# gaetanfacchinetti/DensityFlows.jl

Measured on AMD Instinct MI355X. Metric: forward+logdetJ Msamples/s, d=5 8-layer RealNVP, 1/2/4/8 MI355X, higher is better.
Workload: dtype f32

## Files before the change

### densityflows.jl_amd/csrc/df_uniform_impl.h

```cpp
#pragma once

#include <type_traits>

#include "df_chain_impl.h"

namespace df {
namespace uni {


using impl::lds4;
using impl::mfma4;
using impl::Stager;

__device__ __forceinline__ float relu_fast(float x) {
    return __int_as_float(__builtin_elementwise_max(__float_as_int(x), 0));
}

__device__ __forceinline__ float xgroup_sum(float p) {
    auto a = __builtin_amdgcn_permlane16_swap(__float_as_uint(p), __float_as_uint(p), false, false);
    const float q = __uint_as_float(a[0]) + __uint_as_float(a[1]);
    auto b = __builtin_amdgcn_permlane32_swap(__float_as_uint(q), __float_as_uint(q), false, false);
    return __uint_as_float(b[0]) + __uint_as_float(b[1]);
}


template <int HT, int TT, int KS = 0>
__device__ __forceinline__ void dense_first(const uint8_t* buf, const UNet& N, const float (&xin)[TT][4],
                                            f32x4 (&acc)[TT][HT]) {
    const int lane = threadIdx.x & 63;
    const float* wb = reinterpret_cast<const float*>(buf + N.off_w0) + lane;
    const int ks = KS > 0 ? KS : N.ks;
    if constexpr (KS > 0) {
#pragma unroll
        for (int m = 0; m < HT; ++m) {
            const float w = wb[m * KS * 64];
#pragma unroll
            for (int t = 0; t < TT; ++t) acc[t][m] = mfma4(w, xin[t][0], f32x4{0.f, 0.f, 0.f, 0.f});
        }
#pragma unroll
        for (int r = 1; r < KS; ++r)
#pragma unroll
            for (int m = 0; m < HT; ++m) {
                const float w = wb[(m * KS + r) * 64];
#pragma unroll
                for (int t = 0; t < TT; ++t) acc[t][m] = mfma4(w, xin[t][r], acc[t][m]);
            }
        return;
    }
#pragma unroll
    for (int t = 0; t < TT; ++t)
#pragma unroll
        for (int m = 0; m < HT; ++m) acc[t][m] = f32x4{0.f, 0.f, 0.f, 0.f};
#pragma unroll
    for (int r = 0; r < 4; ++r) {
        if (r < ks) {
#pragma unroll
            for (int m = 0; m < HT; ++m) {
                const float w = wb[(m * ks + r) * 64];
#pragma unroll
                for (int t = 0; t < TT; ++t) acc[t][m] = mfma4(w, xin[t][r], acc[t][m]);
            }
        }
    }
}

template <int HT, int TT>
__device__ __forceinline__ void dense_hidden(const uint8_t* wb, const f32x4 (&in)[TT][HT], f32x4 (&out)[TT][HT]) {
    const int lane = threadIdx.x & 63;
    wb += lane * 16;
    constexpr int MB = HT < 2 ? HT : 2;
#pragma unroll
    for (int t = 0; t < TT; ++t)
#pragma unroll
        for (int m = 0; m < HT; ++m) out[t][m] = f32x4{0.f, 0.f, 0.f, 0.f};
#pragma unroll
    for (int m0 = 0; m0 < HT; m0 += MB) {
        f32x4 w[2][MB];
#pragma unroll
        for (int mm = 0; mm < MB; ++mm) w[0][mm] = lds4(wb + (m0 + mm) * 1024);
#pragma unroll
        for (int kq = 0; kq < HT; ++kq) {
            const int cb = kq & 1;
            if (kq + 1 < HT) {
#pragma unroll
                for (int mm = 0; mm < MB; ++mm) w[cb ^ 1][mm] = lds4(wb + ((kq + 1) * HT + m0 + mm) * 1024);
            }
#pragma unroll
            for (int r = 0; r < 4; ++r)
#pragma unroll
                for (int mm = 0; mm < MB; ++mm)
#pragma unroll
                    for (int t = 0; t < TT; ++t)
                        out[t][m0 + mm] = mfma4(w[cb][mm][r], in[t][kq][r], out[t][m0 + mm]);
        }
    }
}

template <int HT, int TT, bool RELU>
__device__ __forceinline__ void bias_act(const uint8_t* bb, int act, f32x4 (&v)[TT][HT], bool add_bias = true) {
    const int g = (threadIdx.x & 63) >> 4;
    if (add_bias) {
#pragma unroll
        for (int m = 0; m < HT; ++m) {
            const f32x4 b = lds4(bb + ((16 * m + 4 * g) << 2));
#pragma unroll
            for (int t = 0; t < TT; ++t) v[t][m] = v[t][m] + b;
        }
    }
    if (RELU || act == DF_ACT_RELU) {
#pragma unroll
        for (int t = 0; t < TT; ++t)
#pragma unroll
            for (int m = 0; m < HT; ++m)
#pragma unroll
                for (int r = 0; r < 4; ++r) v[t][m][r] = relu_fast(v[t][m][r]);
    } else if (act != DF_ACT_IDENTITY) {
        if (!RELU) {
#pragma unroll
            for (int t = 0; t < TT; ++t)
#pragma unroll
                for (int m = 0; m < HT; ++m)
#pragma unroll
                    for (int r = 0; r < 4; ++r) v[t][m][r] = impl::act_fn(act, v[t][m][r]);
        }
    }
}

template <int HT, int TT, bool RELU, int NO = 0>
__device__ __forceinline__ void out_valu(const uint8_t* buf, const UNet& N, const f32x4 (&h)[TT][HT],
                                         f32x4 (&o)[TT]) {
    const int g = (threadIdx.x & 63) >> 4;
    const uint8_t* w3 = buf + N.off_out;
    constexpr int INP = 16 * HT;
    const int n_out = NO > 0 ? NO : N.n_out;
    const float* b3 = reinterpret_cast<const float*>(w3) + n_out * INP;
#pragma unroll
    for (int t = 0; t < TT; ++t) o[t] = f32x4{0.f, 0.f, 0.f, 0.f};
#pragma unroll
    for (int oo = 0; oo < 4; ++oo) {
        if (oo < n_out) {
            float p[TT];
#pragma unroll
            for (int t = 0; t < TT; ++t) p[t] = 0.f;
#pragma unroll
            for (int kq = 0; kq < HT; ++kq) {
                const f32x4 w = lds4(w3 + ((oo * INP + 16 * kq + 4 * g) << 2));
#pragma unroll
                for (int r = 0; r < 4; ++r)
#pragma unroll
                    for (int t = 0; t < TT; ++t) p[t] = __builtin_fmaf(w[r], h[t][kq][r], p[t]);
            }
            const float bo = b3[oo];
#pragma unroll
            for (int t = 0; t < TT; ++t) {
                const float v = xgroup_sum(p[t]) + bo;
                o[t][oo] = (RELU || N.act_out == DF_ACT_IDENTITY) ? v : impl::act_fn(N.act_out, v);
            }
        }
    }
}

template <int HT, int TT, int NO>
__device__ __forceinline__ void out_valu_t(const uint8_t* buf, const UNet& N, const f32x4 (&h)[TT][HT],
                                           float (&y)[TT]) {
    static_assert(NO >= 1 && NO <= 4, "FAST tails: 1..4 outputs");
    const int g = (threadIdx.x & 63) >> 4;
    const uint8_t* w3 = buf + N.off_out;
    constexpr int INP = 16 * HT;
    float p[TT][4];
#pragma unroll
    for (int t = 0; t < TT; ++t)
#pragma unroll
        for (int oo = 0; oo < 4; ++oo) p[t][oo] = 0.f;
#pragma unroll
    for (int oo = 0; oo < NO; ++oo)
#pragma unroll
        for (int kq = 0; kq < HT; ++kq) {
            const f32x4 w = lds4(w3 + ((oo * INP + 16 * kq + 4 * g) << 2));
#pragma unroll
            for (int r = 0; r < 4; ++r)
#pragma unroll
                for (int t = 0; t < TT; ++t) p[t][oo] = __builtin_fmaf(w[r], h[t][kq][r], p[t][oo]);
        }
    const float bo = reinterpret_cast<const float*>(w3)[NO * INP + (g < NO ? g : 0)];
#pragma unroll
    for (int t = 0; t < TT; ++t) {
        auto a = __builtin_amdgcn_permlane16_swap(__float_as_uint(p[t][0]), __float_as_uint(p[t][1]), false, false);
        const float A = __uint_as_float(a[0]) + __uint_as_float(a[1]);
        float Bv = 0.f;
        if constexpr (NO > 2) {
            auto b = __builtin_amdgcn_permlane16_swap(__float_as_uint(p[t][2]), __float_as_uint(p[t][3]), false, false);
            Bv = __uint_as_float(b[0]) + __uint_as_float(b[1]);
        }
        auto c = __builtin_amdgcn_permlane32_swap(__float_as_uint(A), __float_as_uint(Bv), false, false);
        y[t] = (__uint_as_float(c[0]) + __uint_as_float(c[1])) + bo;
    }
}

template <int NO>
__device__ __forceinline__ float group_row_sum(float y) {
    float s = y;
    if constexpr (NO > 1) {
        auto a = __builtin_amdgcn_permlane16_swap(__float_as_uint(y), __float_as_uint(y), false, false);
        s = s + __uint_as_float(a[1]);
    }
    if constexpr (NO > 2) {
        auto b = __builtin_amdgcn_permlane32_swap(__float_as_uint(y), __float_as_uint(y), false, false);
        const float y2 = __uint_as_float(b[1]);
        s = s + y2;
        if constexpr (NO > 3) {
            auto c = __builtin_amdgcn_permlane16_swap(__float_as_uint(y2), __float_as_uint(y2), false, false);
            s = s + __uint_as_float(c[1]);
        }
    }
    return s;
}

template <int HT, int TT, bool RELU>
__device__ __forceinline__ void out_mfma(const uint8_t* buf, const UNet& N, const f32x4 (&h)[TT][HT],
                                         f32x4 (&out)[TT][2]) {
    const int lane = threadIdx.x & 63, g = lane >> 4;
    const uint8_t* wb = buf + N.off_out + lane * 16;
    const int mt = (N.n_out + 15) >> 4;
#pragma unroll
    for (int t = 0; t < TT; ++t) out[t][0] = out[t][1] = f32x4{0.f, 0.f, 0.f, 0.f};
#pragma unroll
    for (int kq = 0; kq < HT; ++kq) {
        const f32x4 w0 = lds4(wb + (kq * mt + 0) * 1024);
#pragma unroll
        for (int r = 0; r < 4; ++r)
#pragma unroll
            for (int t = 0; t < TT; ++t) out[t][0] = mfma4(w0[r], h[t][kq][r], out[t][0]);
        if (mt > 1) {
            const f32x4 w1 = lds4(wb + (kq * mt + 1) * 1024);
#pragma unroll
            for (int r = 0; r < 4; ++r)
#pragma unroll
                for (int t = 0; t < TT; ++t) out[t][1] = mfma4(w1[r], h[t][kq][r], out[t][1]);
        }
    }
    const uint8_t* bb = buf + N.off_out + HT * mt * 1024;
#pragma unroll
    for (int m = 0; m < 2; ++m) {
        if (m < mt) {
            const f32x4 b = lds4(bb + ((16 * m + 4 * g) << 2));
#pragma unroll
            for (int t = 0; t < TT; ++t) {
                f32x4 v = out[t][m] + b;
                if (!RELU && N.act_out != DF_ACT_IDENTITY)
#pragma unroll
                    for (int r = 0; r < 4; ++r) v[r] = impl::act_fn(N.act_out, v[r]);
                out[t][m] = v;
            }
        }
    }
}

template <int PH>
__device__ __forceinline__ float couple1(float v, float y) {
    if (PH == impl::PH_S_FWD) return v * expf(y);
    if (PH == impl::PH_T_FWD) return v + y;
    if (PH == impl::PH_T_BWD) return v - y;
    return v * expf(-y);
}

template <int HT, int TT, bool OUTV, bool RELU, int PH, int NO = 0>
__device__ __forceinline__ void tail(const uint8_t* buf, const UNet& N, const ULayer& L, const int32_t* tab,
                                     float* state, const int (&ro)[TT], float (&sum)[TT], const f32x4 (&H)[TT][HT]) {
    const int g = (threadIdx.x & 63) >> 4;
    constexpr bool SPH = (PH == impl::PH_S_FWD || PH == impl::PH_S_BWD);
    const int32_t* af = tab + L.af_tab;
    const int n_af = (OUTV && NO > 0) ? NO : L.n_af;
#pragma unroll
    for (int t = 0; t < TT; ++t) sum[t] = 0.f;
#ifdef DF_EXP_NOTAIL
    if (true) {
#pragma unroll
        for (int t = 0; t < TT; ++t) {
            float acc = 0.f;
#pragma unroll
            for (int m = 0; m < HT; ++m) acc += H[t][m][0];
            asm volatile("" ::"v"(acc));
        }
        return;
    }
#endif
    if constexpr (OUTV && NO > 0) {
        float y[TT];
        out_valu_t<HT, TT, NO>(buf, N, H, y);
        const int slot = af[g < NO ? g : 0];
#pragma unroll
        for (int t = 0; t < TT; ++t) {
            if (g < NO) state[ro[t] + slot] = couple1<PH>(state[ro[t] + slot], y[t]);
            if (SPH) sum[t] = group_row_sum<NO>(y[t]);
        }
    } else if constexpr (OUTV) {
        f32x4 o[TT];
        out_valu<HT, TT, RELU, NO>(buf, N, H, o);
        const int slot = (g < n_af) ? af[g] : 0;
#pragma unroll
        for (int t = 0; t < TT; ++t) {
            const float y = impl::sel4(o[t], g);
            if (g < n_af) state[ro[t] + slot] = couple1<PH>(state[ro[t] + slot], y);
            if (SPH) {
                float s_ = o[t][0];
#pragma unroll
                for (int oo = 1; oo < 4; ++oo)
                    if (oo < n_af) s_ = s_ + o[t][oo];
                sum[t] = s_;
            }
        }
    } else {
        f32x4 o[TT][2];
        out_mfma<HT, TT, RELU>(buf, N, H, o);
#pragma unroll
        for (int t = 0; t < TT; ++t) {
            float p = 0.f;
#pragma unroll
            for (int m = 0; m < 2; ++m)
#pragma unroll
                for (int r = 0; r < 4; ++r) {
                    const int oo = 16 * m + 4 * g + r;
                    if (oo < L.n_af) {
                        const int slot = af[oo];
                        const float y = o[t][m][r];
                        state[ro[t] + slot] = couple1<PH>(state[ro[t] + slot], y);
                        if (SPH) p = p + y;
                    }
                }
            if (SPH) sum[t] = xgroup_sum(p);
        }
    }
}

typedef __bf16 bf16x8 __attribute__((ext_vector_type(8)));

__device__ __forceinline__ f32x4 mfma_bf(const bf16x8& a, const bf16x8& b, f32x4 c) {
    return __builtin_amdgcn_mfma_f32_16x16x32_bf16(a, b, c, 0, 0, 0);
}

typedef __bf16 bf16x2 __attribute__((ext_vector_type(2)));
#ifndef DF_SPLIT_DOT2
#define DF_SPLIT_DOT2 1
#endif
template <int S>
__device__ __forceinline__ float split_rem(bf16x2 h, float x) {
#if DF_SPLIT_DOT2 == 2
    const uint32_t u = __builtin_bit_cast(uint32_t, h);
    const float hi = __uint_as_float(S == 0 ? (u << 16) : (u & 0xffff0000u));
    float r;
    asm("v_sub_f32 %0, %1, %2" : "=v"(r) : "v"(x), "v"(hi));
    return r;
#elif DF_SPLIT_DOT2
    uint32_t c;
    if (S == 0) asm("v_mov_b32 %0, 0xbf80" : "=v"(c));
    else c = 0xbf800000u;
    return __builtin_amdgcn_fdot2_f32_bf16(h, __builtin_bit_cast(bf16x2, c), x, false);
#else
    return x - (float)h[S];
#endif
}

__device__ __forceinline__ void split2(float a, float b, bf16x2& p0, bf16x2& p1, bf16x2& p2) {
    p0 = bf16x2{(__bf16)a, (__bf16)b};
    const float ra = split_rem<0>(p0, a), rb = split_rem<1>(p0, b);
    p1 = bf16x2{(__bf16)ra, (__bf16)rb};
    p2 = bf16x2{(__bf16)split_rem<0>(p1, ra), (__bf16)split_rem<1>(p1, rb)};
}

__device__ __forceinline__ void split8(const float (&v)[8], bf16x8& p0, bf16x8& p1, bf16x8& p2) {
#pragma unroll
    for (int e = 0; e < 8; e += 2) {
        bf16x2 h, m, l;
        split2(v[e], v[e + 1], h, m, l);
        p0[e] = h[0]; p0[e + 1] = h[1];
        p1[e] = m[0]; p1[e + 1] = m[1];
        p2[e] = l[0]; p2[e + 1] = l[1];
    }
}

#ifndef DF_SPLIT_MREM
#define DF_SPLIT_MREM 1
#endif
typedef short short4v __attribute__((ext_vector_type(4)));
typedef __bf16 bf16x4v __attribute__((ext_vector_type(4)));

__device__ __forceinline__ short4v neg_eye() {
    const int i = threadIdx.x & 3;
    short4v p;
#pragma unroll
    for (int e = 0; e < 4; ++e) p[e] = (e == i) ? (short)0xbf80 : (short)0;
    return p;
}

__device__ __forceinline__ f32x4 mrem(short4v eye, bf16x4v h, f32x4 c) {
    return __builtin_amdgcn_mfma_f32_4x4x4bf16_1k(eye, __builtin_bit_cast(short4v, h), c, 0, 0, 0);
}

__device__ __forceinline__ void split8_mrem(short4v eye, const f32x4& a, const f32x4& b, bf16x8& p0, bf16x8& p1,
                                            bf16x8& p2) {
    bf16x4v h0, h1;
#pragma unroll
    for (int e = 0; e < 4; ++e) {
        h0[e] = (__bf16)a[e];
        h1[e] = (__bf16)b[e];
    }
    p0 = __builtin_shufflevector(h0, h1, 0, 1, 2, 3, 4, 5, 6, 7);
    const f32x4 ra = mrem(eye, h0, a), rb = mrem(eye, h1, b);
#pragma unroll
    for (int e = 0; e < 4; ++e) {
        h0[e] = (__bf16)ra[e];
        h1[e] = (__bf16)rb[e];
    }
    p1 = __builtin_shufflevector(h0, h1, 0, 1, 2, 3, 4, 5, 6, 7);
    const f32x4 sa = mrem(eye, h0, ra), sb = mrem(eye, h1, rb);
#pragma unroll
    for (int e = 0; e < 4; ++e) {
        h0[e] = (__bf16)sa[e];
        h1[e] = (__bf16)sb[e];
    }
    p2 = __builtin_shufflevector(h0, h1, 0, 1, 2, 3, 4, 5, 6, 7);
}

template <int HT, int TT>
__device__ __forceinline__ void dense_first_split(const uint8_t* buf, const UNet& N, const float (&xin)[TT][4],
                                                  f32x4 (&acc)[TT][HT]) {
    const int lane = threadIdx.x & 63;
    bf16x8 b[TT];
    const __bf16 z = (__bf16)0.f;
#pragma unroll
    for (int t = 0; t < TT; t += 2) {
        bf16x2 h, m, l;
        split2(xin[t][0], t + 1 < TT ? xin[t + 1][0] : 0.f, h, m, l);
        b[t] = bf16x8{h[0], m[0], h[0], l[0], m[0], h[0], z, z};
        if (t + 1 < TT) b[t + 1] = bf16x8{h[1], m[1], h[1], l[1], m[1], h[1], z, z};
    }
    const uint8_t* wb = buf + N.off_w0 + lane * 16;
#pragma unroll
    for (int m = 0; m < HT; ++m) {
        const bf16x8 w = *reinterpret_cast<const bf16x8*>(wb + m * 1024);
#pragma unroll
        for (int t = 0; t < TT; ++t) acc[t][m] = mfma_bf(w, b[t], f32x4{0.f, 0.f, 0.f, 0.f});
    }
}

template <int HT, int TT, bool BIAS = true, bool FENCE = false>
__device__ __forceinline__ void dense_hidden_split(const uint8_t* wb, const f32x4 (&in)[TT][HT],
                                                   f32x4 (&out)[TT][HT]) {
    const int lane = threadIdx.x & 63, g = lane >> 4;
    const uint8_t* bb = wb + (HT / 2) * HT * 3072;
    wb += lane * 16;
    const short4v eye = DF_SPLIT_MREM ? neg_eye() : short4v{0, 0, 0, 0};
#pragma unroll
    for (int m = 0; m < HT; ++m) {
        const f32x4 b = BIAS ? lds4(bb + ((16 * m + 4 * g) << 2)) : f32x4{0.f, 0.f, 0.f, 0.f};
#pragma unroll
        for (int t = 0; t < TT; ++t) out[t][m] = b;
    }
#pragma unroll
    for (int c = 0; c < HT / 2; ++c) {
        bf16x8 x[TT][3];
#pragma unroll
        for (int t = 0; t < TT; ++t) {
            const float v[8] = {in[t][2 * c][0],     in[t][2 * c][1],     in[t][2 * c][2],     in[t][2 * c][3],
                                in[t][2 * c + 1][0], in[t][2 * c + 1][1], in[t][2 * c + 1][2], in[t][2 * c + 1][3]};
#ifdef DF_DIAG_NOSPLIT
            for (int e = 0; e < 8; ++e) x[t][0][e] = (__bf16)v[e];
            x[t][1] = x[t][0];
            x[t][2] = x[t][0];
#else
            if constexpr (DF_SPLIT_MREM) split8_mrem(eye, in[t][2 * c], in[t][2 * c + 1], x[t][0], x[t][1], x[t][2]);
            else split8(v, x[t][0], x[t][1], x[t][2]);
#endif
        }
#pragma unroll
        for (int m = 0; m < HT; ++m) {
            const uint8_t* f = wb + (c * HT + m) * 3072;
            const bf16x8 w0 = *reinterpret_cast<const bf16x8*>(f);
            const bf16x8 w1 = *reinterpret_cast<const bf16x8*>(f + 1024);
            const bf16x8 w2 = *reinterpret_cast<const bf16x8*>(f + 2048);
#pragma unroll
            for (int t = 0; t < TT; ++t) {
                f32x4 a = out[t][m];
                a = mfma_bf(w2, x[t][0], a);
                a = mfma_bf(w1, x[t][1], a);
                a = mfma_bf(w0, x[t][2], a);
                a = mfma_bf(w1, x[t][0], a);
                a = mfma_bf(w0, x[t][1], a);
                out[t][m] = mfma_bf(w0, x[t][0], a);
            }
            if (FENCE) asm volatile("" ::: "memory");
        }
    }
}

#ifndef DF_SPLIT_PREFETCH
#define DF_SPLIT_PREFETCH 1
#endif

__device__ __forceinline__ void sched_fence() { __builtin_amdgcn_sched_barrier(0); }

__device__ __forceinline__ void lds_wait0() { __builtin_amdgcn_s_waitcnt(0xc07f); }

struct SplitStep {
    bf16x8 w0, w1, w2;
    f32x4 b;
};

template <int HT, bool BIAS>
__device__ __forceinline__ void split_step_request(const uint8_t* wl, const uint8_t* bl, int s, SplitStep& f) {
    if (s >= (HT / 2) * HT) return;
    const uint8_t* p = wl + s * 3072;
    f.w0 = *reinterpret_cast<const bf16x8*>(p);
    f.w1 = *reinterpret_cast<const bf16x8*>(p + 1024);
    f.w2 = *reinterpret_cast<const bf16x8*>(p + 2048);
    if (BIAS && s < HT) f.b = lds4(bl + (s << 6));
}

template <int HT, int TT, bool BIAS = true>
__device__ __forceinline__ void dense_hidden_split_pf(const uint8_t* wb, int lane, const f32x4 (&in)[TT][HT],
                                                      f32x4 (&out)[TT][HT], const SplitStep& f0) {
    const int g = lane >> 4;
    const uint8_t* bl = wb + (HT / 2) * HT * 3072 + (g << 4);
    const uint8_t* wl = wb + lane * 16;
    const short4v eye = neg_eye();
    SplitStep f[2];
    f[0] = f0;
    bf16x8 x[TT][3];
#pragma unroll
    for (int s = 0; s < (HT / 2) * HT; ++s) {
        const int c = s / HT, m = s % HT;
        if (m == 0) {
#pragma unroll
            for (int t = 0; t < TT; ++t) split8_mrem(eye, in[t][2 * c], in[t][2 * c + 1], x[t][0], x[t][1], x[t][2]);
        }
        constexpr int NS = (HT / 2) * HT;
        const bool late = (m == HT - 1) && (s + 1 < NS);
        sched_fence();
        lds_wait0();
        if (!late) split_step_request<HT, BIAS>(wl, bl, s + 1, f[(s + 1) & 1]);
        sched_fence();
        const SplitStep& w = f[s & 1];
#pragma unroll
        for (int t = 0; t < TT; ++t) {
            f32x4 a = c == 0 ? (BIAS ? w.b : f32x4{0.f, 0.f, 0.f, 0.f}) : out[t][m];
            a = mfma_bf(w.w2, x[t][0], a);
            a = mfma_bf(w.w1, x[t][1], a);
            a = mfma_bf(w.w0, x[t][2], a);
            a = mfma_bf(w.w1, x[t][0], a);
            a = mfma_bf(w.w0, x[t][1], a);
            out[t][m] = mfma_bf(w.w0, x[t][0], a);
        }
        if (late) {
#pragma unroll
            for (int t = 0; t < TT; ++t) asm volatile("" : "+v"(out[t][m]));
            sched_fence();
            split_step_request<HT, BIAS>(wl, bl, s + 1, f[(s + 1) & 1]);
        }
    }
}

template <int HT, int TT>
__device__ __forceinline__ void dense_first_split_pf(const bf16x8 (&w)[HT], const float (&xin)[TT][4],
                                                     f32x4 (&acc)[TT][HT]) {
    bf16x8 b[TT];
    const __bf16 z = (__bf16)0.f;
#pragma unroll
    for (int t = 0; t < TT; t += 2) {
        bf16x2 h, m, l;
        split2(xin[t][0], t + 1 < TT ? xin[t + 1][0] : 0.f, h, m, l);
        b[t] = bf16x8{h[0], m[0], h[0], l[0], m[0], h[0], z, z};
        if (t + 1 < TT) b[t + 1] = bf16x8{h[1], m[1], h[1], l[1], m[1], h[1], z, z};
    }
#pragma unroll
    for (int m = 0; m < HT; ++m)
#pragma unroll
        for (int t = 0; t < TT; ++t) acc[t][m] = mfma_bf(w[m], b[t], f32x4{0.f, 0.f, 0.f, 0.f});
}

template <int HT, int NO>
__device__ __forceinline__ void out_row_request(const uint8_t* w3g, int oo, f32x4 (&w)[HT]) {
    if (oo >= NO) return;
#pragma unroll
    for (int kq = 0; kq < HT; ++kq) w[kq] = lds4(w3g + ((oo * 16 * HT + 16 * kq) << 2));
}

template <int HT, int TT, int NO>
__device__ __forceinline__ void out_valu_t_pf(const uint8_t* w3g, const f32x4 (&w0)[HT], float bo,
                                              const f32x4 (&h)[TT][HT], const float* state, const int (&ro)[TT],
                                              const int& aslot, float (&v)[TT], float (&y)[TT]) {
    static_assert(NO >= 1 && NO <= 4, "FAST tails: 1..4 outputs");
    float p[TT][4];
#pragma unroll
    for (int t = 0; t < TT; ++t)
#pragma unroll
        for (int oo = 0; oo < 4; ++oo) p[t][oo] = 0.f;
    f32x4 w[2][HT];
#pragma unroll
    for (int kq = 0; kq < HT; ++kq) w[0][kq] = w0[kq];
#pragma unroll
    for (int oo = 0; oo < NO; ++oo) {
        sched_fence();
        lds_wait0();
        if (oo == 0) {
#pragma unroll
            for (int t = 0; t < TT; ++t) v[t] = state[ro[t] + aslot];
        }
        out_row_request<HT, NO>(w3g, oo + 1, w[(oo + 1) & 1]);
        sched_fence();
#pragma unroll
        for (int kq = 0; kq < HT; ++kq)
#pragma unroll
            for (int r = 0; r < 4; ++r)
#pragma unroll
                for (int t = 0; t < TT; ++t) p[t][oo] = __builtin_fmaf(w[oo & 1][kq][r], h[t][kq][r], p[t][oo]);
#pragma unroll
        for (int t = 0; t < TT; ++t) asm volatile("" : "+v"(p[t][oo]));
    }
#pragma unroll
    for (int t = 0; t < TT; ++t) {
        auto a = __builtin_amdgcn_permlane16_swap(__float_as_uint(p[t][0]), __float_as_uint(p[t][1]), false, false);
        const float A = __uint_as_float(a[0]) + __uint_as_float(a[1]);
        float Bv = 0.f;
        if constexpr (NO > 2) {
            auto b = __builtin_amdgcn_permlane16_swap(__float_as_uint(p[t][2]), __float_as_uint(p[t][3]), false, false);
            Bv = __uint_as_float(b[0]) + __uint_as_float(b[1]);
        }
        auto c = __builtin_amdgcn_permlane32_swap(__float_as_uint(A), __float_as_uint(Bv), false, false);
        y[t] = (__uint_as_float(c[0]) + __uint_as_float(c[1])) + bo;
    }
}

struct SplitHead {
    int off_w0, feat_word, af_word;
};
#if DF_SPLIT_PREFETCH && !defined(DF_EXP_NOTAIL) && !defined(DF_DIAG_NOSPLIT)
#define DF_SPLIT_HEAD_REGS 1
#else
#define DF_SPLIT_HEAD_REGS 0
#endif

#ifndef DF_SPLIT_PRIO
#define DF_SPLIT_PRIO 1
#endif
template <bool MATRIX_PHASE>
__device__ __forceinline__ void split_prio() {
    if constexpr (DF_SPLIT_PRIO == 1) __builtin_amdgcn_s_setprio(MATRIX_PHASE ? 2 : 0);
    if constexpr (DF_SPLIT_PRIO == 2) __builtin_amdgcn_s_setprio(MATRIX_PHASE ? 0 : 2);
}

template <int HT, int TT, bool OUTV, bool RELU, int PH, bool FAST = false, int NO = 0, bool SPLIT = false>
__device__ __forceinline__ void net_tiles(const uint8_t* buf, const UNet& N, const ULayer& L, const int32_t* tab,
                                          float* state, const int (&ro)[TT], float (&sum)[TT], const SplitHead& hd) {
    const int lane = threadIdx.x & 63, g = lane >> 4;
    constexpr bool SPH = (PH == impl::PH_S_FWD || PH == impl::PH_S_BWD);
#if DF_SPLIT_HEAD_REGS
    if constexpr (SPLIT && FAST && HT >= 2 && OUTV && NO > 0) {
        int tx = threadIdx.x;
        asm volatile("" : "+v"(tx));
        const int lane = tx & 63, g = lane >> 4;
        const uint8_t* net = buf + hd.off_w0;
        const int slot = ((uint32_t)hd.feat_word >> (kSplitSlotBits * g)) & ((1 << kSplitSlotBits) - 1);
        bf16x8 w0[HT];
#pragma unroll
        for (int m = 0; m < HT; ++m) w0[m] = *reinterpret_cast<const bf16x8*>(net + lane * 16 + m * 1024);
        float xin[TT][4];
#pragma unroll
        for (int t = 0; t < TT; ++t) xin[t][0] = state[ro[t] + slot];
        const uint8_t* wh = net + kSplitOffH(HT);
        SplitStep f0;
        split_step_request<HT, true>(wh + lane * 16, wh + (HT / 2) * HT * 3072 + (g << 4), 0, f0);
        sched_fence();
        lds_wait0();
        split_prio<true>();
        sched_fence();
        f32x4 A[TT][HT], B[TT][HT];
        dense_first_split_pf<HT, TT>(w0, xin, A);
        bias_act<HT, TT, true>(buf, DF_ACT_RELU, A, false);
        dense_hidden_split_pf<HT, TT>(wh, lane, A, B, f0);
        const uint8_t* w3 = net + kSplitOffOut(HT);
        const uint8_t* w3g = w3 + (g << 4);
        sched_fence();
        split_prio<false>();
        f32x4 wo[HT];
        out_row_request<HT, NO>(w3g, 0, wo);
        const float bo = reinterpret_cast<const float*>(w3)[NO * 16 * HT + (g < NO ? g : 0)];
        const int aslot = ((uint32_t)hd.af_word >> (kSplitSlotBits * g)) & ((1 << kSplitSlotBits) - 1);
        sched_fence();
        bias_act<HT, TT, true>(buf, DF_ACT_RELU, B, false);
        float v[TT], y[TT];
        out_valu_t_pf<HT, TT, NO>(w3g, wo, bo, B, state, ro, aslot, v, y);
#pragma unroll
        for (int t = 0; t < TT; ++t) {
            if (g < NO) state[ro[t] + aslot] = couple1<PH>(v[t], y[t]);
            sum[t] = SPH ? group_row_sum<NO>(y[t]) : 0.f;
        }
        return;
    }
#endif
    if constexpr (SPLIT && FAST && HT >= 2) {
        float xin[TT][4];
        const int slot = tab[L.feat_tab + g];
#pragma unroll
        for (int t = 0; t < TT; ++t) xin[t][0] = state[ro[t] + slot];
        f32x4 A[TT][HT], B[TT][HT];
        dense_first_split<HT, TT>(buf, N, xin, A);
        bias_act<HT, TT, true>(buf, DF_ACT_RELU, A, false);
        dense_hidden_split<HT, TT>(buf + N.off_h, A, B);
        bias_act<HT, TT, true>(buf, DF_ACT_RELU, B, false);
        tail<HT, TT, OUTV, RELU, PH, NO>(buf, N, L, tab, state, ro, sum, B);
        return;
    }
    float xin[TT][4];
    const int32_t* feat = tab + L.feat_tab;
    constexpr int KS = FAST ? 1 : 0;
    const int ks = FAST ? 1 : N.ks;
#pragma unroll
    for (int r = 0; r < 4; ++r) {
        const int slot = (r < ks) ? feat[4 * r + g] : 0;
#pragma unroll
        for (int t = 0; t < TT; ++t) xin[t][r] = (r < ks) ? state[ro[t] + slot] : 0.f;
    }

    f32x4 A[TT][HT], B[TT][HT];
    dense_first<HT, TT, KS>(buf, N, xin, A);
    bias_act<HT, TT, RELU>(buf + N.off_b0, N.act0, A, FAST ? false : !N.fold0);
    if (FAST || N.nh == 1) {
        dense_hidden<HT, TT>(buf + N.off_h, A, B);
        bias_act<HT, TT, RELU>(buf + N.off_h + HT * HT * 1024, N.acth, B);
        tail<HT, TT, OUTV, RELU, PH, NO>(buf, N, L, tab, state, ro, sum, B);
        return;
    }
    bool in_a = true;
    for (int k = 0; k < N.nh; k += 2) {
        dense_hidden<HT, TT>(buf + N.off_h + k * N.hstride, A, B);
        bias_act<HT, TT, RELU>(buf + N.off_h + k * N.hstride + HT * HT * 1024, N.acth, B);
        in_a = false;
        if (k + 1 < N.nh) {
            dense_hidden<HT, TT>(buf + N.off_h + (k + 1) * N.hstride, B, A);
            bias_act<HT, TT, RELU>(buf + N.off_h + (k + 1) * N.hstride + HT * HT * 1024, N.acth, A);
            in_a = true;
        }
    }
    if (in_a) tail<HT, TT, OUTV, RELU, PH, NO>(buf, N, L, tab, state, ro, sum, A);
    else tail<HT, TT, OUTV, RELU, PH, NO>(buf, N, L, tab, state, ro, sum, B);
}

template <int HT, int TT, bool RELU, bool FWDP, int NO>
__device__ __forceinline__ void net_pair_tiles(const uint8_t* buf, const ULayer& L, const int32_t* tab, float* state,
                                               const int (&ro)[TT], float (&ssum)[TT]) {
    const int lane = threadIdx.x & 63, g = lane >> 4;
    float xin[TT][4];
    const int slot_in = tab[L.feat_tab + g];
#pragma unroll
    for (int t = 0; t < TT; ++t) xin[t][0] = state[ro[t] + slot_in];
    f32x4 As[TT][HT], At[TT][HT], Bs[TT][HT], Bt[TT][HT];
    dense_first<HT, TT, 1>(buf, L.s, xin, As);
    dense_first<HT, TT, 1>(buf, L.t, xin, At);
    bias_act<HT, TT, RELU>(buf + L.s.off_b0, L.s.act0, As, false);
    bias_act<HT, TT, RELU>(buf + L.t.off_b0, L.t.act0, At, false);
    dense_hidden<HT, TT>(buf + L.s.off_h, As, Bs);
    dense_hidden<HT, TT>(buf + L.t.off_h, At, Bt);
    bias_act<HT, TT, RELU>(buf + L.s.off_h + HT * HT * 1024, L.s.acth, Bs);
    bias_act<HT, TT, RELU>(buf + L.t.off_h + HT * HT * 1024, L.t.acth, Bt);
    float ys[TT], yt[TT];
    out_valu_t<HT, TT, NO>(buf, L.s, Bs, ys);
    out_valu_t<HT, TT, NO>(buf, L.t, Bt, yt);
    const int slot = tab[L.af_tab + (g < NO ? g : 0)];
#pragma unroll
    for (int t = 0; t < TT; ++t) {
        if (g < NO) {
            float v = state[ro[t] + slot];
            if (FWDP) {
                v = v * expf(ys[t]);
                v = v + yt[t];
            } else {
                v = v - yt[t];
                v = v * expf(-ys[t]);
            }
            state[ro[t] + slot] = v;
        }
        ssum[t] = group_row_sum<NO>(ys[t]);
    }
}

}

#ifndef DF_UNI_WAVES
#define DF_UNI_WAVES 4
#endif
#ifndef DF_FAST_WAVES
#define DF_FAST_WAVES 4
#endif

template <int HT, int MODE, bool OUTV, bool RELU, bool FAST = false, bool SPLIT = false>
__global__ void __launch_bounds__(kBlockThreads, FAST ? DF_FAST_WAVES : DF_UNI_WAVES)
uniform_kernel(ChainArgs a) {
    using namespace uni;
    constexpr bool FWD = (MODE == MODE_FWD || MODE == MODE_FWD_INPLACE);
    constexpr bool WANT_LDJ = (MODE != MODE_FWD_INPLACE);

    extern __shared__ __attribute__((aligned(16))) uint8_t smem[];
    const int stage_area = a.stage_bytes * a.n_stage_bufs;
    int32_t* tab = reinterpret_cast<int32_t*>(smem + stage_area);
    float* state = reinterpret_cast<float*>(smem + stage_area + a.tab_bytes);

    ClockStamp clk;
    clk.begin(a);
#ifdef DF_PHASE_STAMPS
    uint64_t ph[16] = {};
#define DF_PH(i) do { if (blockIdx.x == 0 && threadIdx.x == 0) ph[i] = __builtin_amdgcn_s_memtime(); } while (0)
#else
#define DF_PH(i) do {} while (0)
#endif
    DF_PH(0);
    const int tid = threadIdx.x;
    const int lane = tid & 63, wave = tid >> 6;
    const int g = lane >> 4, j = lane & 15;
    const int d = a.d, n = a.n, stride = a.stride, nd = n + d;
    const int nt = a.tiles;
    const int S = kWavesPerBlock * 16 * nt;
    const int cA = nd + 1, cE = nd + 2;
    const int64_t s0 = (int64_t)blockIdx.x * S;
    const int nvalid = (int)((a.batch - s0) < S ? (a.batch - s0) : S);

    Stager sg;
    sg.base = smem;
    sg.bytes = a.stage_bytes;
    sg.sched = FWD ? a.sched_fwd : a.sched_bwd;
    sg.n = FWD ? a.n_sched_fwd : a.n_sched_bwd;
    constexpr bool kLaneLocalDma = SPLIT && DF_SPLIT_PREFETCH;
    constexpr bool kSplitHead = SPLIT && FAST && OUTV && HT >= 2 && DF_SPLIT_HEAD_REGS;
    impl::stager_start<kLaneLocalDma>(sg, a);

    float* tabf = reinterpret_cast<float*>(tab);
    constexpr int kRowMax = 8;
    const bool fast_copy = d <= kRowMax && n <= kRowMax && a.n_par <= kBlockThreads && a.tab_ints <= 4 * kBlockThreads;
    auto row_init = [&](int smp) {
        for (int c = nd; c < stride; ++c) state[smp * stride + c] = (c == nd + 3) ? 1.f : 0.f;
    };
    auto theta_in = [&](float v, float lo, float hi) {
        const float diff = hi - lo;
        return (diff == 0.f) ? 0.f : (v - lo) / diff;
    };
    if (fast_copy) {
        const int n_tab = a.tab_ints, n_par = a.n_par;
        int tv[4];
#pragma unroll
        for (int u = 0; u < 4; ++u) {
            const int i = tid + u * kBlockThreads;
            tv[u] = i < n_tab ? a.tables[i] : 0;
        }
        const float pv = tid < n_par ? a.params[tid] : 0.f;
        const bool norm_th = a.tmin != nullptr;
        const float blo = (norm_th && lane < n) ? a.tmin[lane] : 0.f;
        const float bhi = (norm_th && lane < n) ? a.tmax[lane] : 0.f;
        const int smp = tid;
        const bool valid = smp < nvalid;
        float zr[kRowMax], tr[kRowMax];
#pragma unroll
        for (int c = 0; c < kRowMax; ++c)
            if (c < d) zr[c] = valid ? a.zin[(s0 + smp) * d + c] : 0.f;
#pragma unroll
        for (int c = 0; c < kRowMax; ++c)
            if (c < n) tr[c] = valid ? a.theta[(s0 + smp) * n + c] : 0.f;
#pragma unroll
        for (int u = 0; u < 4; ++u) {
            const int i = tid + u * kBlockThreads;
            if (i < n_tab) tab[i] = tv[u];
        }
        if (tid < n_par) tabf[n_tab + tid] = pv;
#pragma unroll
        for (int c = 0; c < kRowMax; ++c)
            if (c < n) {
                const float lo = __shfl(blo, c), hi = __shfl(bhi, c);
                if (smp < S) state[smp * stride + c] = (norm_th && valid) ? theta_in(tr[c], lo, hi) : tr[c];
            }
        if (smp < S) {
#pragma unroll
            for (int c = 0; c < kRowMax; ++c)
                if (c < d) state[smp * stride + n + c] = zr[c];
            row_init(smp);
        }
        for (int i = tid + kBlockThreads * d; i < S * d; i += kBlockThreads) {
            const int r = i / d, c = i - r * d;
            state[r * stride + n + c] = r < nvalid ? a.zin[(s0 + r) * d + c] : 0.f;
        }
        for (int i = tid + kBlockThreads * n; i < S * n; i += kBlockThreads) {
            const int r = i / n, c = i - r * n;
            float v = 0.f;
            if (r < nvalid) {
                v = a.theta[(s0 + r) * n + c];
                if (norm_th) v = theta_in(v, a.tmin[c], a.tmax[c]);
            }
            state[r * stride + c] = v;
        }
        for (int r = tid + kBlockThreads; r < S; r += kBlockThreads) row_init(r);
    } else {
        for (int i = tid; i < a.tab_ints; i += kBlockThreads) tab[i] = a.tables[i];
        for (int i = tid; i < S * d; i += kBlockThreads) {
            const int smp = i / d, c = i - smp * d;
            float v = 0.f;
            if (smp < nvalid) v = a.zin[(s0 + smp) * d + c];
            state[smp * stride + n + c] = v;
        }
        for (int i = tid; i < S * n; i += kBlockThreads) {
            const int smp = i / n, c = i - smp * n;
            float v = 0.f;
            if (smp < nvalid) {
                v = a.theta[(s0 + smp) * n + c];
                if (a.tmin) v = theta_in(v, a.tmin[c], a.tmax[c]);
            }
            state[smp * stride + c] = v;
        }
        for (int i = tid; i < S; i += kBlockThreads) row_init(i);
    }
    DF_PH(1);
    DF_PH(2);
    DF_PH(3);
    __syncthreads();
    DF_PH(4);

    const int row0 = ((wave * nt) * 16 + j) * stride;
#ifdef DF_NO_PAIR
    constexpr bool no_pair = true;
#else
    constexpr bool no_pair = false;
#endif
    const int tstep = 16 * stride;
    bool have_acc = false;

    auto ldj_update = [&](int ro, float l, bool first_in_elem, bool last_in_elem) {
        if (!WANT_LDJ || g != 0) return;
        const float e = first_in_elem ? l : state[ro + cE] + l;
        state[ro + cE] = e;
        if (last_in_elem) state[ro + cA] = have_acc ? state[ro + cA] + e : e;
    };

    for (int it = 0; it < a.n_layers; ++it) {
        const int li = FWD ? it : a.n_layers - 1 - it;
        using CULayer = const __attribute__((address_space(4))) ULayer;
#ifdef DF_PHASE_STAMPS
        const ULayer L = *(const ULayer*)(&((CULayer*)(uintptr_t)a.ulayers)[li]);
        asm volatile("s_waitcnt lgkmcnt(0)" ::: "memory");
        if (it == 1) DF_PH(13);
#else
        const ULayer& L = *(const ULayer*)(&((CULayer*)(uintptr_t)a.ulayers)[li]);
#endif
        const int kind = L.kind;
        const bool first_in_elem = FWD ? L.elem_start : L.elem_end;
        const bool last_in_elem = FWD ? L.elem_end : L.elem_start;
        int gl = g, jl = j, wavel = wave, row0l = row0;
        if constexpr (kLaneLocalDma) {
            if (kind == DF_LAYER_NORM || (!FWD && a.snap)) {
                int tx = tid;
                asm volatile("" : "+v"(tx));
                gl = (tx & 63) >> 4, jl = tx & 15, wavel = tx >> 6;
                row0l = ((wavel * nt) * 16 + jl) * stride;
            }
        }
        if (kind == DF_LAYER_NORM) {
            const float al = L.alpha, be = L.beta, delta = be - al;
            auto norm = [&](const auto* xmn) {
                const auto* xmx = xmn + d;
                for (int tt = 0; tt < nt; ++tt) {
                    const int ro = row0l + tt * tstep;
                    for (int i = gl; i < d; i += 4) {
                        const float lo = xmn[i], hi = xmx[i], xd = hi - lo;
                        float v = state[ro + n + i];
                        if (FWD) v = ((xd * v - al * hi) + be * lo) / delta;
                        else v = (be * (v - lo) + al * (hi - v)) / xd;
                        state[ro + n + i] = v;
                    }
                    ldj_update(ro, FWD ? L.ldj_const : -L.ldj_const, first_in_elem, last_in_elem);
                }
            };
            if (fast_copy) norm(tabf + a.tab_ints + L.norm_off);
            else norm(a.params + L.norm_off);
        } else {
            const bool rnvp = (kind == DF_LAYER_RNVP);
            constexpr int kTT = FAST ? kFastTileGroup : kUniformTileGroup;
            auto tiles_loop = [&](const UNet& N, const SplitHead& hd, auto ph_tag, auto no_tag, bool sphase,
                                  float sign) {
                constexpr int PH = decltype(ph_tag)::value;
                constexpr int NO = decltype(no_tag)::value;
                const uint8_t* buf = sg.buf();
                for (int tt = 0; tt < nt; tt += kTT) {
                    int ro[kTT];
                    float ssum[kTT];
                    int r0 = row0;
                    if constexpr (SPLIT) asm volatile("" : "+v"(r0));
#pragma unroll
                    for (int t = 0; t < kTT; ++t) ro[t] = r0 + (tt + t) * tstep;
                    net_tiles<HT, kTT, OUTV, RELU, PH, FAST, NO, SPLIT>(buf, N, L, tab, state, ro, ssum, hd);
#pragma unroll
                    for (int t = 0; t < kTT; ++t) {
                        if (sphase) ldj_update(ro[t], sign * ssum[t], first_in_elem, last_in_elem);
                        else if (!rnvp) ldj_update(ro[t], 0.f, first_in_elem, last_in_elem);
                    }
                }
            };
            auto run_net = [&](const UNet& N, auto ph_tag, bool sphase, float sign) {
                SplitHead hd{0, 0, 0};
                int stage = N.stage, n_out = N.n_out;
                if constexpr (kSplitHead) {
                    hd = SplitHead{N.off_w0, L.feat_word, L.af_word};
                    asm volatile("" : "+s"(stage), "+s"(n_out), "+s"(hd.off_w0), "+s"(hd.feat_word), "+s"(hd.af_word));
                }
                impl::ensure_stage<kLaneLocalDma>(stage, sg, a);
                if constexpr (FAST && OUTV) {
                    switch (n_out) {
                        case 1: tiles_loop(N, hd, ph_tag, std::integral_constant<int, 1>{}, sphase, sign); break;
                        case 2: tiles_loop(N, hd, ph_tag, std::integral_constant<int, 2>{}, sphase, sign); break;
                        case 3: tiles_loop(N, hd, ph_tag, std::integral_constant<int, 3>{}, sphase, sign); break;
                        default: tiles_loop(N, hd, ph_tag, std::integral_constant<int, 4>{}, sphase, sign); break;
                    }
                } else {
                    tiles_loop(N, hd, ph_tag, std::integral_constant<int, 0>{}, sphase, sign);
                }
            };
            using PSF = std::integral_constant<int, impl::PH_S_FWD>;
            using PTF = std::integral_constant<int, impl::PH_T_FWD>;
            using PTB = std::integral_constant<int, impl::PH_T_BWD>;
            using PSB = std::integral_constant<int, impl::PH_S_BWD>;
            bool paired = false;
            if constexpr (FAST && OUTV && !SPLIT && HT <= 2) {
                if (rnvp && L.s.stage == L.t.stage && L.s.n_out == L.t.n_out && !no_pair) {
                    impl::ensure_stage(L.s.stage, sg, a);
                    auto pair_loop = [&](auto no_tag) {
                        constexpr int NO = decltype(no_tag)::value;
                        const uint8_t* buf = sg.buf();
                        for (int tt = 0; tt < nt; tt += kTT) {
                            int ro[kTT];
                            float ssum[kTT];
#pragma unroll
                            for (int t = 0; t < kTT; ++t) ro[t] = row0 + (tt + t) * tstep;
                            net_pair_tiles<HT, kTT, RELU, FWD, NO>(buf, L, tab, state, ro, ssum);
#pragma unroll
                            for (int t = 0; t < kTT; ++t)
                                ldj_update(ro[t], FWD ? ssum[t] : -ssum[t], first_in_elem, last_in_elem);
                        }
                    };
                    switch (L.s.n_out) {
                        case 1: pair_loop(std::integral_constant<int, 1>{}); break;
                        case 2: pair_loop(std::integral_constant<int, 2>{}); break;
                        case 3: pair_loop(std::integral_constant<int, 3>{}); break;
                        default: pair_loop(std::integral_constant<int, 4>{}); break;
                    }
                    paired = true;
                }
            }
            if (paired) {
            } else if (FWD) {
#ifdef DF_PHASE_STAMPS
                if (it == 1) DF_PH(11);
#endif
                if (rnvp) run_net(L.s, PSF{}, true, 1.f);
#ifdef DF_PHASE_STAMPS
                if (it == 1) DF_PH(12);
#endif
                run_net(L.t, PTF{}, false, 1.f);
            } else {
                run_net(L.t, PTB{}, false, 1.f);
                if (rnvp) run_net(L.s, PSB{}, true, -1.f);
            }
        }
        have_acc = have_acc || last_in_elem;
#ifdef DF_PHASE_STAMPS
        if (it == 0) DF_PH(5);
        if (it == 1) DF_PH(6);
        if (it == 2) DF_PH(7);
        if (it == 3) DF_PH(8);
#endif
        if (!FWD && a.snap) {
            float* dst = a.snap + (int64_t)li * a.batch * d;
            for (int tt = 0; tt < nt; ++tt) {
                const int smp = (wavel * nt + tt) * 16 + jl;
                if (smp < nvalid)
                    for (int i = gl; i < d; i += 4) dst[(s0 + smp) * d + i] = state[row0l + tt * tstep + n + i];
            }
        }
    }

    asm volatile("s_waitcnt vmcnt(0)" ::: "memory");
    if (MODE == MODE_LOGPDF) {
        double part = 0.0;
        if (g == 0) {
            for (int tt = 0; tt < nt; ++tt) {
                const int ro = row0 + tt * tstep;
                const int smp = (wave * nt + tt) * 16 + j;
                float q = 0.f;
                for (int i = 0; i < d; ++i) {
                    const float zz = state[ro + n + i];
                    q = q + zz * zz;
                }
                const float lp = (a.c0 - q / 2.f) + state[ro + cA];
                if (smp < nvalid) {
                    if (a.lp_out) a.lp_out[s0 + smp] = lp;
                    part += (double)lp;
                }
            }
        }
        if (a.partial) {
#pragma unroll
            for (int off = 32; off >= 1; off >>= 1) part += __shfl_xor(part, off);
            __syncthreads();
            double* red = reinterpret_cast<double*>(smem);
            if (lane == 0) red[wave] = part;
            __syncthreads();
            if (tid == 0) {
                double s = 0.0;
                for (int w = 0; w < kWavesPerBlock; ++w) s += red[w];
                a.partial[blockIdx.x] = s;
            }
        }
        if (!a.xout) {
            clk.end(a);
            return;
        }
    }
    __syncthreads();
    for (int i = tid; i < S * d; i += kBlockThreads) {
        const int smp = i / d, c = i - smp * d;
        if (smp < nvalid) a.xout[(s0 + smp) * d + c] = state[smp * stride + n + c];
    }
    if (WANT_LDJ && MODE != MODE_LOGPDF && a.ldj_out) {
        for (int i = tid; i < nvalid; i += kBlockThreads) a.ldj_out[s0 + i] = state[i * stride + cA];
    }
    DF_PH(9);
#ifdef DF_PHASE_STAMPS
    asm volatile("s_waitcnt vmcnt(0)" ::: "memory");
    DF_PH(10);
    if (blockIdx.x == 0 && threadIdx.x == 0) {
#pragma unroll
        for (int i = 1; i < 14; ++i) a.xout[i] = (float)(ph[i] - ph[0]);
    }
#endif
#undef DF_PH
    clk.end(a);
}

template <int HT, bool RELU, bool FAST = false, bool SPLIT = false>
void* uniform_kernel_ptr_r(int mode, bool outv) {
#define DF_U(M) (outv ? reinterpret_cast<void*>(&uniform_kernel<HT, M, true, RELU, FAST, SPLIT>) \
                      : reinterpret_cast<void*>(&uniform_kernel<HT, M, false, RELU, FAST, SPLIT>))
    switch (mode) {
        case MODE_FWD: return DF_U(MODE_FWD);
        case MODE_FWD_INPLACE: return DF_U(MODE_FWD_INPLACE);
        case MODE_BWD: return DF_U(MODE_BWD);
        default: return DF_U(MODE_LOGPDF);
    }
#undef DF_U
}

template <int HT>
void* uniform_kernel_ptr(int mode, int variant) {
    const bool outv = variant & 1;
    if constexpr (HT >= 2) {
        if ((variant & 8) && (variant & 4) && outv) return uniform_kernel_ptr_r<HT, true, true, true>(mode, true);
    }
    if (variant & 8) return nullptr;
    if (variant & 4) return uniform_kernel_ptr_r<HT, true, true>(mode, outv);
    return (variant & 2) ? uniform_kernel_ptr_r<HT, true>(mode, outv) : uniform_kernel_ptr_r<HT, false>(mode, outv);
}

template <int HT>
hipError_t launch_uniform_ht(int mode, int variant, const ChainArgs& a, unsigned grid, size_t lds, hipStream_t st) {
    void* args[] = {const_cast<ChainArgs*>(&a)};
    return hipLaunchKernel(uniform_kernel_ptr<HT>(mode, variant), dim3(grid), dim3(kBlockThreads), args, lds, st);
}

template <int HT>
hipError_t set_uniform_lds_limit_ht(size_t lds) {
    for (int mode = 0; mode < 4; ++mode)
        for (int v = 0; v < 16; ++v) {
            void* k = uniform_kernel_ptr<HT>(mode, v);
            if (!k) continue;
            hipError_t e = hipFuncSetAttribute(k,
                                               hipFuncAttributeMaxDynamicSharedMemorySize, (int)lds);
            if (e != hipSuccess) return e;
        }
    return hipSuccess;
}

template <int HT>
hipError_t uniform_occupancy_ht(int mode, int variant, size_t lds, int* blocks) {
    return hipOccupancyMaxActiveBlocksPerMultiprocessor(blocks, uniform_kernel_ptr<HT>(mode, variant), kBlockThreads,
                                                        lds);
}

}
```

Baseline: 1735.

## Split output tail across lane groups and prefetch logdet state in split path

For TT=2 with one or two outputs, each 16-lane group now owns a single row/output pair. A single permlane reduction tree then serves both tiles, instead of running a full reduction per tile with idle groups. The logdet accumulator reads (e_old, a_old) move into the output phase alongside the coupling read, so their latency overlaps the VALU dot products, and all lane groups write the logdet rather than only group 0. Lane byte offsets are precomputed and held in VGPRs, and the first-layer split is made per tile. The cost is extra template plumbing and an assumption about the slot-bit layout, which a static_assert guards.

```diff
diff --git a/densityflows.jl_amd/csrc/df_uniform_impl.h b/densityflows.jl_amd/csrc/df_uniform_impl.h
--- a/densityflows.jl_amd/csrc/df_uniform_impl.h
+++ b/densityflows.jl_amd/csrc/df_uniform_impl.h
@@ -518,11 +518,10 @@
 }
 
 template <int HT, int TT, bool BIAS = true>
-__device__ __forceinline__ void dense_hidden_split_pf(const uint8_t* wb, int lane, const f32x4 (&in)[TT][HT],
+__device__ __forceinline__ void dense_hidden_split_pf(const uint8_t* wb, int l16, int g16, const f32x4 (&in)[TT][HT],
                                                       f32x4 (&out)[TT][HT], const SplitStep& f0) {
-    const int g = lane >> 4;
-    const uint8_t* bl = wb + (HT / 2) * HT * 3072 + (g << 4);
-    const uint8_t* wl = wb + lane * 16;
+    const uint8_t* bl = wb + (HT / 2) * HT * 3072 + g16;
+    const uint8_t* wl = wb + l16;
     const short4v eye = neg_eye();
     SplitStep f[2];
     f[0] = f0;
@@ -566,11 +565,13 @@
     bf16x8 b[TT];
     const __bf16 z = (__bf16)0.f;
 #pragma unroll
-    for (int t = 0; t < TT; t += 2) {
+    for (int t = 0; t < TT; ++t) {
         bf16x2 h, m, l;
-        split2(xin[t][0], t + 1 < TT ? xin[t + 1][0] : 0.f, h, m, l);
+        h = bf16x2{(__bf16)xin[t][0], z};
+        const float r1 = split_rem<0>(h, xin[t][0]);
+        m = bf16x2{(__bf16)r1, z};
+        l = bf16x2{(__bf16)split_rem<0>(m, r1), z};
         b[t] = bf16x8{h[0], m[0], h[0], l[0], m[0], h[0], z, z};
-        if (t + 1 < TT) b[t + 1] = bf16x8{h[1], m[1], h[1], l[1], m[1], h[1], z, z};
     }
 #pragma unroll
     for (int m = 0; m < HT; ++m)
@@ -585,11 +586,21 @@
     for (int kq = 0; kq < HT; ++kq) w[kq] = lds4(w3g + ((oo * 16 * HT + 16 * kq) << 2));
 }
 
-template <int HT, int TT, int NO>
+constexpr int split_tail_rows(int TT, int NO) { return (TT == 2 && NO <= 2) ? 1 : TT; }
+
+template <int TT>
+struct SplitTail {
+    int ce, l16, g16;
+    int row[TT];
+    float e_old[TT], a_old[TT];
+};
+
+template <int HT, int TT, int NO, bool LDJ, int NU>
 __device__ __forceinline__ void out_valu_t_pf(const uint8_t* w3g, const f32x4 (&w0)[HT], float bo,
-                                              const f32x4 (&h)[TT][HT], const float* state, const int (&ro)[TT],
-                                              const int& aslot, float (&v)[TT], float (&y)[TT]) {
+                                              const f32x4 (&h)[TT][HT], const float* state, const int& aslot,
+                                              SplitTail<TT>& tl, float (&v)[NU], float (&y)[NU]) {
     static_assert(NO >= 1 && NO <= 4, "FAST tails: 1..4 outputs");
+    static_assert(NU == split_tail_rows(TT, NO), "rows a lane group owns");
     float p[TT][4];
 #pragma unroll
     for (int t = 0; t < TT; ++t)
@@ -604,7 +615,13 @@
         lds_wait0();
         if (oo == 0) {
 #pragma unroll
-            for (int t = 0; t < TT; ++t) v[t] = state[ro[t] + aslot];
+            for (int u = 0; u < NU; ++u) {
+                v[u] = state[tl.row[u] + aslot];
+                if constexpr (LDJ) {
+                    tl.e_old[u] = state[tl.row[u] + tl.ce];
+                    tl.a_old[u] = state[tl.row[u] + tl.ce - 1];
+                }
+            }
         }
         out_row_request<HT, NO>(w3g, oo + 1, w[(oo + 1) & 1]);
         sched_fence();
@@ -617,17 +634,30 @@
 #pragma unroll
         for (int t = 0; t < TT; ++t) asm volatile("" : "+v"(p[t][oo]));
     }
-#pragma unroll
-    for (int t = 0; t < TT; ++t) {
-        auto a = __builtin_amdgcn_permlane16_swap(__float_as_uint(p[t][0]), __float_as_uint(p[t][1]), false, false);
+    if constexpr (NU < TT) {
+        const float q = NO == 2 ? p[0][1] : p[1][0];
+        auto a = __builtin_amdgcn_permlane16_swap(__float_as_uint(p[0][0]), __float_as_uint(q), false, false);
         const float A = __uint_as_float(a[0]) + __uint_as_float(a[1]);
-        float Bv = 0.f;
-        if constexpr (NO > 2) {
-            auto b = __builtin_amdgcn_permlane16_swap(__float_as_uint(p[t][2]), __float_as_uint(p[t][3]), false, false);
+        float Bv = A;
+        if constexpr (NO == 2) {
+            auto b = __builtin_amdgcn_permlane16_swap(__float_as_uint(p[1][0]), __float_as_uint(p[1][1]), false, false);
             Bv = __uint_as_float(b[0]) + __uint_as_float(b[1]);
         }
         auto c = __builtin_amdgcn_permlane32_swap(__float_as_uint(A), __float_as_uint(Bv), false, false);
-        y[t] = (__uint_as_float(c[0]) + __uint_as_float(c[1])) + bo;
+        y[0] = (__uint_as_float(c[0]) + __uint_as_float(c[1])) + bo;
+    } else {
+#pragma unroll
+        for (int t = 0; t < TT; ++t) {
+            auto a = __builtin_amdgcn_permlane16_swap(__float_as_uint(p[t][0]), __float_as_uint(p[t][1]), false, false);
+            const float A = __uint_as_float(a[0]) + __uint_as_float(a[1]);
+            float Bv = 0.f;
+            if constexpr (NO > 2) {
+                auto b = __builtin_amdgcn_permlane16_swap(__float_as_uint(p[t][2]), __float_as_uint(p[t][3]), false, false);
+                Bv = __uint_as_float(b[0]) + __uint_as_float(b[1]);
+            }
+            auto c = __builtin_amdgcn_permlane32_swap(__float_as_uint(A), __float_as_uint(Bv), false, false);
+            y[t] = (__uint_as_float(c[0]) + __uint_as_float(c[1])) + bo;
+        }
     }
 }
 
@@ -649,27 +679,34 @@
     if constexpr (DF_SPLIT_PRIO == 2) __builtin_amdgcn_s_setprio(MATRIX_PHASE ? 0 : 2);
 }
 
-template <int HT, int TT, bool OUTV, bool RELU, int PH, bool FAST = false, int NO = 0, bool SPLIT = false>
+template <int HT, int TT, bool OUTV, bool RELU, int PH, bool FAST = false, int NO = 0, bool SPLIT = false,
+          bool LDJ = false, bool LANES = false>
 __device__ __forceinline__ void net_tiles(const uint8_t* buf, const UNet& N, const ULayer& L, const int32_t* tab,
-                                          float* state, const int (&ro)[TT], float (&sum)[TT], const SplitHead& hd) {
+                                          float* state, const int (&ro)[TT], float (&sum)[TT], const SplitHead& hd,
+                                          SplitTail<TT>& tl) {
     const int lane = threadIdx.x & 63, g = lane >> 4;
     constexpr bool SPH = (PH == impl::PH_S_FWD || PH == impl::PH_S_BWD);
 #if DF_SPLIT_HEAD_REGS
     if constexpr (SPLIT && FAST && HT >= 2 && OUTV && NO > 0) {
-        int tx = threadIdx.x;
-        asm volatile("" : "+v"(tx));
-        const int lane = tx & 63, g = lane >> 4;
+        int l16 = tl.l16, g16 = tl.g16;
+        if constexpr (!LANES) {
+            int tx = threadIdx.x;
+            asm volatile("" : "+v"(tx));
+            l16 = (tx & 63) << 4, g16 = tx & 48;
+        }
+        const int g = g16 >> 4;
         const uint8_t* net = buf + hd.off_w0;
-        const int slot = ((uint32_t)hd.feat_word >> (kSplitSlotBits * g)) & ((1 << kSplitSlotBits) - 1);
+        const int slot = ((uint32_t)hd.feat_word >> (g16 >> 1)) & ((1 << kSplitSlotBits) - 1);
+        static_assert(kSplitSlotBits == 8, "slot of lane group g at bit 8 g = g16 / 2");
         bf16x8 w0[HT];
 #pragma unroll
-        for (int m = 0; m < HT; ++m) w0[m] = *reinterpret_cast<const bf16x8*>(net + lane * 16 + m * 1024);
+        for (int m = 0; m < HT; ++m) w0[m] = *reinterpret_cast<const bf16x8*>(net + l16 + m * 1024);
         float xin[TT][4];
 #pragma unroll
         for (int t = 0; t < TT; ++t) xin[t][0] = state[ro[t] + slot];
         const uint8_t* wh = net + kSplitOffH(HT);
         SplitStep f0;
-        split_step_request<HT, true>(wh + lane * 16, wh + (HT / 2) * HT * 3072 + (g << 4), 0, f0);
+        split_step_request<HT, true>(wh + l16, wh + (HT / 2) * HT * 3072 + g16, 0, f0);
         sched_fence();
         lds_wait0();
         split_prio<true>();
@@ -677,23 +714,44 @@
         f32x4 A[TT][HT], B[TT][HT];
         dense_first_split_pf<HT, TT>(w0, xin, A);
         bias_act<HT, TT, true>(buf, DF_ACT_RELU, A, false);
-        dense_hidden_split_pf<HT, TT>(wh, lane, A, B, f0);
+        dense_hidden_split_pf<HT, TT>(wh, l16, g16, A, B, f0);
         const uint8_t* w3 = net + kSplitOffOut(HT);
-        const uint8_t* w3g = w3 + (g << 4);
+        const uint8_t* w3g = w3 + g16;
         sched_fence();
         split_prio<false>();
         f32x4 wo[HT];
         out_row_request<HT, NO>(w3g, 0, wo);
-        const float bo = reinterpret_cast<const float*>(w3)[NO * 16 * HT + (g < NO ? g : 0)];
-        const int aslot = ((uint32_t)hd.af_word >> (kSplitSlotBits * g)) & ((1 << kSplitSlotBits) - 1);
+        constexpr int NU = split_tail_rows(TT, NO);
+        constexpr bool ONE_TREE = NU < TT;
+        const int go = ONE_TREE ? (NO == 2 ? (g & 1) : 0) : (g < NO ? g : 0);
+        const float bo = reinterpret_cast<const float*>(w3)[NO * 16 * HT + go];
+        const int aslot = ((uint32_t)hd.af_word >> (kSplitSlotBits * go)) & ((1 << kSplitSlotBits) - 1);
+        if constexpr (ONE_TREE) {
+            tl.row[0] = ro[0] + ((NO == 2 ? (g >> 1) : (g & 1)) ? ro[1] - ro[0] : 0);
+        } else {
+#pragma unroll
+            for (int t = 0; t < TT; ++t) tl.row[t] = ro[t];
+        }
         sched_fence();
         bias_act<HT, TT, true>(buf, DF_ACT_RELU, B, false);
-        float v[TT], y[TT];
-        out_valu_t_pf<HT, TT, NO>(w3g, wo, bo, B, state, ro, aslot, v, y);
-#pragma unroll
-        for (int t = 0; t < TT; ++t) {
-            if (g < NO) state[ro[t] + aslot] = couple1<PH>(v[t], y[t]);
-            sum[t] = SPH ? group_row_sum<NO>(y[t]) : 0.f;
+        float v[NU], y[NU];
+        out_valu_t_pf<HT, TT, NO, SPH && LDJ>(w3g, wo, bo, B, state, aslot, tl, v, y);
+        if (ONE_TREE || g < NO) {
+#pragma unroll
+            for (int u = 0; u < NU; ++u) state[tl.row[u] + aslot] = couple1<PH>(v[u], y[u]);
+        }
+#pragma unroll
+        for (int u = 0; u < NU; ++u) {
+            if constexpr (!SPH) {
+                sum[u] = 0.f;
+            } else if constexpr (ONE_TREE && NO == 2) {
+                auto a = __builtin_amdgcn_permlane16_swap(__float_as_uint(y[u]), __float_as_uint(y[u]), false, false);
+                sum[u] = __uint_as_float(a[0]) + __uint_as_float(a[1]);
+            } else if constexpr (ONE_TREE) {
+                sum[u] = y[u];
+            } else {
+                sum[u] = group_row_sum<NO>(y[u]);
+            }
         }
         return;
     }
@@ -929,6 +987,9 @@
 #endif
     const int tstep = 16 * stride;
     bool have_acc = false;
+    constexpr bool kHoldLanes = kSplitHead && HT == 4 && FWD;
+    int lane16 = lane << 4, group16 = g << 4;
+    if constexpr (kHoldLanes) asm volatile("" : "+v"(lane16), "+v"(group16));
 
     auto ldj_update = [&](int ro, float l, bool first_in_elem, bool last_in_elem) {
         if (!WANT_LDJ || g != 0) return;
@@ -992,11 +1053,30 @@
                     if constexpr (SPLIT) asm volatile("" : "+v"(r0));
 #pragma unroll
                     for (int t = 0; t < kTT; ++t) ro[t] = r0 + (tt + t) * tstep;
-                    net_tiles<HT, kTT, OUTV, RELU, PH, FAST, NO, SPLIT>(buf, N, L, tab, state, ro, ssum, hd);
-#pragma unroll
-                    for (int t = 0; t < kTT; ++t) {
-                        if (sphase) ldj_update(ro[t], sign * ssum[t], first_in_elem, last_in_elem);
-                        else if (!rnvp) ldj_update(ro[t], 0.f, first_in_elem, last_in_elem);
+                    SplitTail<kTT> tl;
+                    tl.ce = cE, tl.l16 = lane16, tl.g16 = group16;
+                    net_tiles<HT, kTT, OUTV, RELU, PH, FAST, NO, SPLIT, WANT_LDJ, kHoldLanes>(buf, N, L, tab, state, ro,
+                                                                                              ssum, hd, tl);
+                    constexpr bool SPH = (PH == impl::PH_S_FWD || PH == impl::PH_S_BWD);
+                    if constexpr (kSplitHead && NO > 0 && SPH) {
+                        constexpr int NU = split_tail_rows(kTT, NO);
+                        if constexpr (WANT_LDJ) {
+                            if (NU < kTT || g == 0) {
+#pragma unroll
+                                for (int u = 0; u < NU; ++u) {
+                                    const float l = sign * ssum[u];
+                                    const float e = first_in_elem ? l : tl.e_old[u] + l;
+                                    state[tl.row[u] + cE] = e;
+                                    if (last_in_elem) state[tl.row[u] + cA] = have_acc ? tl.a_old[u] + e : e;
+                                }
+                            }
+                        }
+                    } else {
+#pragma unroll
+                        for (int t = 0; t < kTT; ++t) {
+                            if (sphase) ldj_update(ro[t], sign * ssum[t], first_in_elem, last_in_elem);
+                            else if (!rnvp) ldj_update(ro[t], 0.f, first_in_elem, last_in_elem);
+                        }
                     }
                 }
             };
```

Result: faster. 1754, median of 6 (+1.1%).
